# Jaureguy760/HaploHyped-VarAwareML

Hardware: AMD Instinct MI355X
Metric: variants/sec encode+compress, 3M-variant x 2.5k-sample VCF (higher is better)
Workload: dtype u8

## Files before the change

### haplohyped_varawareml_amd/csrc/api.hip

```cpp
#include "common.h"
#include <chrono>
#include <vector>
#include <stdarg.h>
#include <stdio.h>
#include <string.h>
#include <stdlib.h>

static thread_local char g_err[512] = "";

void hhgt_set_error(const char *fmt, ...)
{
    va_list ap;
    va_start(ap, fmt);
    vsnprintf(g_err, sizeof(g_err), fmt, ap);
    va_end(ap);
}

extern "C" const char *hhgt_last_error(void) { return g_err; }
extern "C" const char *hhgt_version(void) { return "hhgt 0.1 (gfx950)"; }

extern "C" int hhgt_device_count(void)
{
    int n = 0;
    if (hipGetDeviceCount(&n) != hipSuccess) return 0;
    return n;
}

int DevBuf::ensure(size_t bytes)
{
    if (bytes <= cap) return HHGT_OK;
    if (p) {
        hipFree(p);
        p = nullptr;
        cap = 0;
    }
    size_t want = bytes + bytes / 8 + 256;
    static const bool dbg = getenv("HHGT_ALLOC_DEBUG") != nullptr;
    const auto t0 = std::chrono::steady_clock::now();
    hipError_t e = hipMalloc(&p, want);
    if (dbg)
        fprintf(stderr, "[alloc] %.3f ms  hipMalloc %zu took %.3f ms\n", std::chrono::duration<double>(t0.time_since_epoch()).count() * 1e3,
                want, std::chrono::duration<double>(std::chrono::steady_clock::now() - t0).count() * 1e3);
    if (e != hipSuccess) {
        p = nullptr;
        hhgt_set_error("hipMalloc(%zu) failed: %s", want, hipGetErrorString(e));
        return HHGT_ERR_HIP;
    }
    cap = want;
    return HHGT_OK;
}

void DevBuf::release()
{
    if (p) hipFree(p);
    p = nullptr;
    cap = 0;
}

#define TRY(expr)                      \
    do {                               \
        int _rc = (expr);              \
        if (_rc != HHGT_OK) return _rc; \
    } while (0)

int EncodeWs::ensure_index(uint32_t n_regions)
{
    TRY(slots.ensure((size_t)n_regions * INDEX_CAP * 4));
    TRY(counts.ensure((size_t)n_regions * 4));
    TRY(prefix.ensure(((size_t)n_regions + 1) * 4));
    return ensure_scan(n_regions);
}

int EncodeWs::ensure_lines(uint32_t max_lines)
{
    const size_t nl4 = ((size_t)max_lines + 1) * 4;
    TRY(nl.ensure(nl4));
    TRY(ensure_scan(max_lines));
    for (DevBuf &b : line) TRY(b.ensure(nl4));
    return ensure_runs();
}

int EncodeWs::ensure_scan(uint64_t n) { return scan_tmp.ensure(2 * scan_tmp_elems(n) * 4); }

int EncodeWs::ensure_runs()
{
    TRY(run_first.ensure(MAX_CHROM_RUNS * 8));
    TRY(run_names.ensure(MAX_CHROM_RUNS * 32));
    return result.ensure(sizeof(hhgt_encode_result));
}

int hhgt_ctx::CodecWs::ensure(uint64_t n_chunks, uint32_t nblocks, uint32_t nwaves, size_t slot)
{
    const uint64_t n_streams = n_chunks * nblocks * nwaves;
    TRY(lz_scratch.ensure((size_t)n_streams * slot));
    TRY(lz_csize.ensure((size_t)n_streams * 4));
    TRY(fr_bsize.ensure((size_t)n_chunks * nblocks * 4));
    TRY(fr_csize.ensure(((size_t)n_chunks + 1) * 8));
    return fr_flags.ensure((size_t)n_chunks * 4);
}

template <typename Launch>
static int timed(hhgt_ctx *c, hipStream_t st, int stage, Launch launch)
{
    StageTimer t(c, st, stage);
    TRY(launch());
    t.stop();
    return HHGT_OK;
}

extern "C" int hhgt_ctx_create(int device, hhgt_ctx **out)
{
    if (!out) return HHGT_ERR_ARG;
    *out = nullptr;
    int n = hhgt_device_count();
    if (n <= 0 || device < 0 || device >= n) {
        hhgt_set_error("no usable HIP device (count=%d, requested=%d): libhhgt has no CPU path", n, device);
        return HHGT_ERR_NO_DEVICE;
    }
    HIP_TRY(hipSetDevice(device));
    hhgt_ctx *c = new hhgt_ctx();
    c->device = device;
    int rc = HHGT_OK;
    hipError_t e = hipGetDeviceProperties(&c->prop, device);
    if (e != hipSuccess) {
        hhgt_set_error("hipGetDeviceProperties failed: %s", hipGetErrorString(e));
        rc = HHGT_ERR_HIP;
    } else if (strncmp(c->prop.gcnArchName, "gfx950", 6) != 0) {
        hhgt_set_error("device %d is %s; libhhgt carries gfx950 code objects only", device, c->prop.gcnArchName);
        rc = HHGT_ERR_NO_DEVICE;
    }
    if (rc == HHGT_OK && (e = hipHostMalloc(reinterpret_cast<void **>(&c->h_counters), sizeof(DevCounters), hipHostMallocDefault)) != hipSuccess) {
        hhgt_set_error("hipHostMalloc failed: %s", hipGetErrorString(e));
        rc = HHGT_ERR_HIP;
    }
    if (rc == HHGT_OK && (e = hipHostMalloc(reinterpret_cast<void **>(&c->h_result_pinned), sizeof(hhgt_encode_result), hipHostMallocDefault)) != hipSuccess) {
        hhgt_set_error("hipHostMalloc failed: %s", hipGetErrorString(e));
        rc = HHGT_ERR_HIP;
    }
    if (rc == HHGT_OK) rc = c->counters.ensure(sizeof(DevCounters));
    if (rc != HHGT_OK) {
        hhgt_ctx_destroy(c);
        return rc;
    }
    *out = c;
    return HHGT_OK;
}

extern "C" void hhgt_ctx_destroy(hhgt_ctx *c)
{
    if (!c) return;
    hipSetDevice(c->device);
    hipDeviceSynchronize();
    c->enc.each([](DevBuf &b) { b.release(); });
    DevBuf *bufs[] = {&c->counters, &c->cursor, &c->dec_bad, &c->oh_ovl, &c->oh_lut, &c->crc_x2n, &c->ld_bits};
    for (DevBuf *b : bufs) b->release();
    for (auto &w : c->cw) {
        DevBuf *wb[] = {&w.lz_scratch, &w.lz_csize, &w.lz_flags, &w.fr_bsize, &w.fr_csize, &w.fr_flags};
        for (DevBuf *b : wb) b->release();
        if (w.lz_done) hipEventDestroy(w.lz_done);
        if (w.fr_done) hipEventDestroy(w.fr_done);
    }
    if (c->h_counters) hipHostFree(c->h_counters);
    if (c->h_result_pinned) hipHostFree(c->h_result_pinned);
    for (auto &p : c->pending) {
        hipEventDestroy(p.a);
        hipEventDestroy(p.b);
    }
    for (auto e : c->event_pool) hipEventDestroy(e);
    delete c;
}

static hipEvent_t get_event(hhgt_ctx *c)
{
    if (!c->event_pool.empty()) {
        hipEvent_t e = c->event_pool.back();
        c->event_pool.pop_back();
        return e;
    }
    hipEvent_t e;
    hipEventCreate(&e);
    return e;
}

StageTimer::StageTimer(hhgt_ctx *c, hipStream_t s, int stage_) : ctx(c), st(s), stage(stage_)
{
    if (ctx->profiling) {
        a = get_event(ctx);
        b = get_event(ctx);
        hipEventRecord(a, st);
    }
}

void StageTimer::stop()
{
    if (a) {
        hipEventRecord(b, st);
        ctx->pending.push_back({stage, a, b});
        a = b = nullptr;
    }
}

int hhgt_profile_collect(hhgt_ctx *c)
{
    for (auto &p : c->pending) {
        hipEventSynchronize(p.b);
        float ms = 0.f;
        if (hipEventElapsedTime(&ms, p.a, p.b) == hipSuccess) {
            c->stage_ms[p.stage] += ms;
            c->stage_launches[p.stage] += 1;
        }
        c->event_pool.push_back(p.a);
        c->event_pool.push_back(p.b);
    }
    c->pending.clear();
    return HHGT_OK;
}

extern "C" int hhgt_profile_enable(hhgt_ctx *c, int on)
{
    if (!c) return HHGT_ERR_ARG;
    c->profiling = on ? 1 : 0;
    return HHGT_OK;
}

extern "C" int hhgt_profile_reset(hhgt_ctx *c)
{
    if (!c) return HHGT_ERR_ARG;
    hhgt_profile_collect(c);
    for (int i = 0; i < HHGT_N_STAGES; ++i) {
        c->stage_ms[i] = 0;
        c->stage_launches[i] = 0;
    }
    return HHGT_OK;
}

extern "C" int hhgt_profile_read(hhgt_ctx *c, double *ms, uint64_t *launches)
{
    if (!c) return HHGT_ERR_ARG;
    hhgt_profile_collect(c);
    for (int i = 0; i < HHGT_N_STAGES; ++i) {
// ... 513 lines not shown
}

static int effective_blocksize(uint64_t chunk_nbytes, int typesize, int blocksize)
{
    if ((uint64_t)blocksize > chunk_nbytes) {
        blocksize = (int)chunk_nbytes;
        if (typesize > 1 && blocksize >= typesize) blocksize -= blocksize % typesize;
    }
    return blocksize > 0 ? blocksize : 1;
}

static int check_decode_block(int typesize, int blocksize)
{
    if (blocksize > 65536) {
        hhgt_set_error("decode: block of %d bytes x typesize %d does not fit LDS (blocks of at most 65536 bytes)",
                       blocksize, typesize);
        return HHGT_ERR_ARG;
    }
    return HHGT_OK;
}

static void codec_geometry(uint64_t chunk_nbytes, int typesize, int blocksize, uint32_t *nblocks, uint32_t *nwaves,
                           size_t *slot_bytes)
{
    const bool split = typesize >= 2 && typesize <= 16 && blocksize / typesize >= 128;
    *nblocks = (uint32_t)((chunk_nbytes + blocksize - 1) / blocksize);
    *nwaves = split ? (uint32_t)typesize : 1u;
    size_t max_stream = split ? (size_t)blocksize / typesize : (size_t)blocksize;
    if (split && chunk_nbytes % blocksize && chunk_nbytes % blocksize > max_stream) max_stream = chunk_nbytes % blocksize;
    *slot_bytes = lz4_slot_bytes((int)max_stream);
}

extern "C" uint64_t hhgt_compress_bound(uint64_t n_chunks, uint64_t chunk_nbytes, int typesize, int blocksize)
{
    if (check_codec_args(chunk_nbytes, typesize, blocksize, HHGT_BLOSC2) != HHGT_OK) return 0;
    return n_chunks * (chunk_nbytes + 32);
}

static int compress_impl(hhgt_ctx *c, const void *d_src, const void *d_planes, PlanesGeom pg, uint64_t n_chunks, uint64_t chunk_nbytes,
                         int typesize, int blocksize, int format, void *d_dst, uint64_t dst_cap,
                         uint64_t *d_chunk_off, uint64_t *total_bytes, void *stream)
{
    if (!c || (!d_src && !d_planes) || !d_dst || !d_chunk_off) return HHGT_ERR_ARG;
    hipStream_t st = reinterpret_cast<hipStream_t>(stream);
    HIP_TRY(hipSetDevice(c->device));
    TRY(check_codec_args(chunk_nbytes, typesize, blocksize, format));
    if (total_bytes) *total_bytes = 0;
    if (n_chunks == 0) return HHGT_OK;
    if (!total_bytes && dst_cap < n_chunks * (chunk_nbytes + 32)) {
        hhgt_set_error("compress: the asynchronous form (total_bytes == NULL) needs dst_cap >= hhgt_compress_bound() = %llu, got %llu",
                       (unsigned long long)(n_chunks * (chunk_nbytes + 32)), (unsigned long long)dst_cap);
        return HHGT_ERR_CAPACITY;
    }
    blocksize = effective_blocksize(chunk_nbytes, typesize, blocksize);
    uint32_t nblocks, nwaves;
    size_t slot;
    codec_geometry(chunk_nbytes, typesize, blocksize, &nblocks, &nwaves, &slot);
    hipStream_t fst = c->frame_stream ? c->frame_stream : st;
    hhgt_ctx::CodecWs &w = c->cw[c->frame_stream ? (c->cmp_seq++ & 1u) : 0u];
    TRY(w.ensure(n_chunks, nblocks, nwaves, slot));
    if (w.fr_pending) {
        HIP_TRY(hipStreamWaitEvent(st, w.fr_done, 0));
        w.fr_pending = false;
    }
    TRY(timed(c, st, HHGT_STAGE_LZ4, [&] {
        if (!w.lz_flags.p) {
            TRY(w.lz_flags.ensure(4));
            HIP_TRY(hipMemsetAsync(w.lz_flags.p, 0, 4, st));
        }
        if (++w.lz_tag == 0) w.lz_tag = 1;
        return launch_lz4_blocks(static_cast<const uint8_t *>(d_src), static_cast<const uint8_t *>(d_planes), pg, n_chunks, chunk_nbytes,
                                 typesize, blocksize, w.lz_scratch.as<uint8_t>(), slot, w.lz_csize.as<uint32_t>(), c->clevel,
                                 w.lz_flags.as<uint32_t>(), w.lz_tag, st);
    }));
    if (fst != st) {
        if (!w.lz_done) HIP_TRY(hipEventCreateWithFlags(&w.lz_done, hipEventDisableTiming));
        if (!w.fr_done) HIP_TRY(hipEventCreateWithFlags(&w.fr_done, hipEventDisableTiming));
        HIP_TRY(hipEventRecord(w.lz_done, st));
        HIP_TRY(hipStreamWaitEvent(fst, w.lz_done, 0));
    }
    TRY(timed(c, fst, HHGT_STAGE_FRAME, [&] {
        return launch_frame(w.lz_scratch.as<uint8_t>(), slot, w.lz_csize.as<uint32_t>(), static_cast<const uint8_t *>(d_src),
                            static_cast<const uint8_t *>(d_planes), pg, n_chunks, chunk_nbytes, typesize, blocksize, format,
                            w.fr_bsize.as<uint32_t>(), w.fr_csize.as<uint64_t>(), static_cast<uint8_t *>(d_dst), dst_cap, d_chunk_off,
                            w.fr_flags.as<uint32_t>(), fst);
    }));
    if (fst != st) {
        HIP_TRY(hipEventRecord(w.fr_done, fst));
        w.fr_pending = true;
        if (total_bytes) HIP_TRY(hipStreamWaitEvent(st, w.fr_done, 0));
    }
    if (total_bytes) {
        uint64_t tot = 0;
        HIP_TRY(hipMemcpyAsync(&tot, d_chunk_off + n_chunks, 8, hipMemcpyDeviceToHost, st));
        HIP_TRY(hipStreamSynchronize(st));
        *total_bytes = tot;
        if (tot > dst_cap) {
            hhgt_set_error("compress: need %llu bytes, dst_cap is %llu", (unsigned long long)tot,
                           (unsigned long long)dst_cap);
            return HHGT_ERR_CAPACITY;
        }
    }
    return HHGT_OK;
}

extern "C" int hhgt_compress_chunks(hhgt_ctx *c, const void *d_src, uint64_t n_chunks, uint64_t chunk_nbytes,
                                    int typesize, int blocksize, int format, void *d_dst, uint64_t dst_cap,
                                    uint64_t *d_chunk_off, uint64_t *total_bytes, void *stream)
{
    if (!d_src) return HHGT_ERR_ARG;
    return compress_impl(c, d_src, nullptr, PlanesGeom{0, 0, 0, 0}, n_chunks, chunk_nbytes, typesize, blocksize, format, d_dst, dst_cap,
                         d_chunk_off, total_bytes, stream);
}

extern "C" int hhgt_compress_planes(hhgt_ctx *c, const hhgt_layout *lay, const void *d_P, const void *d_G, uint32_t col0, uint32_t n_cols,
                                    int format, void *d_dst, uint64_t dst_cap, uint64_t *d_chunk_off, uint64_t *total_bytes,
                                    void *stream)
{
    if (!c || !d_P) return HHGT_ERR_ARG;
    LayoutDev L;
    PlanesGeom pg;
    TRY(planes_columns(lay, col0, n_cols, &L, &pg));
    const uint64_t chunk_nbytes = (uint64_t)L.Sc * L.Vc * 2ull, col_bytes = chunk_nbytes * L.n_sc;
    const uint8_t *g = d_G ? static_cast<const uint8_t *>(d_G) + (uint64_t)col0 * col_bytes : nullptr;
    return compress_impl(c, g, d_P, pg, (uint64_t)n_cols * L.n_sc, chunk_nbytes, 2, 8192, format, d_dst, dst_cap, d_chunk_off, total_bytes,
                         stream);
}

extern "C" int hhgt_reserve(hhgt_ctx *c, uint64_t text_bytes, uint32_t max_lines, uint64_t n_chunks, uint64_t chunk_nbytes, int typesize,
                            int blocksize)
{
    if (!c) return HHGT_ERR_ARG;
    HIP_TRY(hipSetDevice(c->device));
    if (text_bytes) {
        const uint32_t n_regions = index_regions(text_bytes);
        TRY(c->enc.ensure_scan(n_regions > max_lines ? n_regions : max_lines));
        TRY(c->enc.ensure_index(n_regions));
        TRY(c->enc.ensure_lines(max_lines));
    }
    if (n_chunks) {
        TRY(check_codec_args(chunk_nbytes, typesize, blocksize, HHGT_BLOSC2));
        blocksize = effective_blocksize(chunk_nbytes, typesize, blocksize);
        uint32_t nblocks, nwaves;
        size_t slot;
        codec_geometry(chunk_nbytes, typesize, blocksize, &nblocks, &nwaves, &slot);
        TRY(c->cw[0].ensure(n_chunks, nblocks, nwaves, slot));
    }
    return HHGT_OK;
}

extern "C" int hhgt_set_clevel(hhgt_ctx *c, int clevel)
{
    if (!c || clevel < 1 || clevel > 9) {
        hhgt_set_error("clevel must be 1..9");
        return HHGT_ERR_ARG;
    }
    c->clevel = clevel;
    return HHGT_OK;
}

extern "C" int hhgt_stream_create(hhgt_ctx *c, int kind, void **out)
{
    if (!c || !out || (kind != HHGT_STREAM_ENCODE && kind != HHGT_STREAM_COMPRESS && kind != HHGT_STREAM_FRAME)) {
        hhgt_set_error("hhgt_stream_create: bad arguments");
        return HHGT_ERR_ARG;
    }
    HIP_TRY(hipSetDevice(c->device));
    hipStream_t st = nullptr;
// ... 353 lines not shown
```

### haplohyped_varawareml_amd/csrc/common.h

```cpp
#pragma once
#include <hip/hip_runtime.h>
#include <stdint.h>
#include <stddef.h>
#include <string>
#include <vector>
#include "../../include/hhgt.h"

#define HHGT_WAVE 64
#ifdef HHGT_ENC_PRIO
#define HHGT_WAVE_PRIO() __builtin_amdgcn_s_setprio(HHGT_ENC_PRIO)
#else
#define HHGT_WAVE_PRIO()
#endif

#ifdef __HIPCC__
__device__ __forceinline__ uint32_t wave_scan_sum_dpp(uint32_t x, uint32_t lane)
{
    x += (uint32_t)__builtin_amdgcn_update_dpp(0, (int)x, 0x111, 0xf, 0xf, false);
    x += (uint32_t)__builtin_amdgcn_update_dpp(0, (int)x, 0x112, 0xf, 0xf, false);
    x += (uint32_t)__builtin_amdgcn_update_dpp(0, (int)x, 0x114, 0xf, 0xf, false);
    x += (uint32_t)__builtin_amdgcn_update_dpp(0, (int)x, 0x118, 0xf, 0xf, false);
    const uint32_t t0 = (uint32_t)__builtin_amdgcn_readlane((int)x, 15);
    const uint32_t t1 = (uint32_t)__builtin_amdgcn_readlane((int)x, 31) + t0;
    const uint32_t t2 = (uint32_t)__builtin_amdgcn_readlane((int)x, 47) + t1;
// ... 73 lines not shown
    uint32_t bpr;
    uint32_t tpc;
    uint32_t col0;
};
static inline __host__ __device__ uint64_t planes_piece(const PlanesGeom &g, uint64_t col, uint32_t tile, uint32_t kp, uint32_t row)
{
    return ((((col * g.tpc + tile) * 4ull + kp) * g.S_pad) + row) * 32ull;
}
static inline __host__ __device__ PlanesGeom planes_geom(const LayoutDev &L, uint32_t col0)
{
    PlanesGeom g;
    g.S_pad = L.n_sc * L.Sc;
    g.bpr = (uint32_t)(L.Vc >> 12);
    g.tpc = (uint32_t)(L.Vc / PL_TILE);
    g.col0 = col0;
    return g;
}
static inline __host__ __device__ void planes_block(const PlanesGeom &g, uint64_t id, uint64_t *col, uint32_t *row, uint32_t *bi)
{
    const uint64_t per_col = (uint64_t)g.S_pad * g.bpr;
    const uint64_t c = id / per_col;
    const uint32_t rem = (uint32_t)(id - c * per_col);
    *col = g.col0 + c;
    *row = rem / g.bpr;
    *bi = rem - (rem / g.bpr) * g.bpr;
}

struct DevBuf {
    void *p = nullptr;
    size_t cap = 0;
    int ensure(size_t bytes);
    void release();
    template <typename T> T *as() const { return reinterpret_cast<T *>(p); }
};

struct LineCols {
    uint32_t *soff, *lend, *pos, *refalt, *flags, *keep, *kidx, *cnew, *crun;
};
struct KeptCols {
    uint32_t *soff, *lend, *meta, *redo_list, *redo_flag;
    uint64_t *run_first;
    uint8_t *run_names;
};

struct EncodeWs {
    DevBuf slots, counts, prefix, nl, scan_tmp;
    enum { L_SOFF, L_LEND, L_POS, L_REFALT, L_FLAGS, L_KEEP, L_KIDX, L_CNEW, L_CRUN, K_SOFF, K_LEND, K_META, REDO_LIST, REDO_FLAG, N_LINE };
    DevBuf line[N_LINE];
    DevBuf run_first, run_names;
    DevBuf result;
    int ensure_index(uint32_t n_regions);
    int ensure_lines(uint32_t max_lines);
    int ensure_scan(uint64_t n);
    int ensure_runs();
    template <typename F> void each(F f)
    {
        for (DevBuf *b : {&slots, &counts, &prefix, &nl, &scan_tmp, &run_first, &run_names, &result}) f(*b);
        for (DevBuf &b : line) f(b);
    }
    uint32_t *col(int i) const { return line[i].as<uint32_t>(); }
    LineCols line_cols() const
    {
        LineCols l;
        l.soff = col(L_SOFF), l.lend = col(L_LEND), l.pos = col(L_POS), l.refalt = col(L_REFALT), l.flags = col(L_FLAGS);
        l.keep = col(L_KEEP), l.kidx = col(L_KIDX), l.cnew = col(L_CNEW), l.crun = col(L_CRUN);
        return l;
    }
    KeptCols kept_cols() const
    {
        KeptCols k;
        k.soff = col(K_SOFF), k.lend = col(K_LEND), k.meta = col(K_META), k.redo_list = col(REDO_LIST), k.redo_flag = col(REDO_FLAG);
        k.run_first = run_first.as<uint64_t>(), k.run_names = run_names.as<uint8_t>();
        return k;
    }
};

struct hhgt_ctx {
    int device = 0;
    hipDeviceProp_t prop;
    EncodeWs enc;
    DevBuf counters;
    DevBuf cursor;
    struct CodecWs {
        DevBuf lz_scratch, lz_csize, lz_flags, fr_bsize, fr_csize, fr_flags;
        uint32_t lz_tag = 0;
        hipEvent_t lz_done = nullptr, fr_done = nullptr;
        bool fr_pending = false;
        int ensure(uint64_t n_chunks, uint32_t nblocks, uint32_t nwaves, size_t slot);
    } cw[2];
    uint64_t cmp_seq = 0;
    hipStream_t frame_stream = nullptr;
    DevBuf dec_bad, oh_ovl, oh_lut, crc_x2n;
    DevBuf ld_bits;
    bool crc_x2n_ready = false;
    DevCounters *h_counters = nullptr;
    hhgt_encode_result *h_result_pinned = nullptr;
    hhgt_encode_result h_result;
    std::vector<uint64_t> run_first_kept;
    std::vector<std::string> run_names_host;
    int clevel = 5;
    int keep_multi = 0;
    int index_mode = -1;
    bool counters_clean = false;
    int profiling = 0;
    double stage_ms[HHGT_N_STAGES] = {0};
    uint64_t stage_launches[HHGT_N_STAGES] = {0};
    struct Pending { int stage; hipEvent_t a, b; };
    std::vector<Pending> pending;
    std::vector<hipEvent_t> event_pool;
};

struct StageTimer {
    hhgt_ctx *ctx;
    hipStream_t st;
    int stage;
    hipEvent_t a = nullptr, b = nullptr;
    StageTimer(hhgt_ctx *c, hipStream_t s, int stage_);
    void stop();
};
int hhgt_profile_collect(hhgt_ctx *ctx);

int launch_scan_exclusive_u32(const uint32_t *d_in, uint32_t *d_out, uint64_t n, uint32_t *d_tmp,
                              size_t tmp_elems, hipStream_t st);
int launch_scan_exclusive_u32_pair(const uint32_t *in_a, uint32_t *out_a, const uint32_t *in_b, uint32_t *out_b, uint64_t n,
                                   uint32_t *d_tmp, size_t tmp_elems, hipStream_t st);
size_t scan_tmp_elems(uint64_t n);

int launch_index_newlines(const uint8_t *d_text, uint64_t n, uint32_t *d_slots, uint32_t *d_counts,
                          uint32_t n_regions, uint32_t min_line, uint32_t S, int mode, DevCounters *d_cnt, hipStream_t st);
int index_mode_default();
int launch_compact_newlines(const uint32_t *d_slots, const uint32_t *d_counts, const uint32_t *d_prefix,
                            uint32_t n_regions, uint32_t *d_nl, uint32_t max_lines, hipStream_t st);
int launch_parse_fixed(const uint8_t *d_text, uint64_t n, const uint32_t *d_nl, const uint32_t *d_nlines,
                       uint32_t max_lines, const RegionFilter &region, uint32_t S, const LineCols &l, int mode,
                       DevCounters *d_cnt, hipStream_t st);
int launch_compact_kept(const uint8_t *d_text, uint64_t n, const uint32_t *d_nl, const uint32_t *d_nlines, uint32_t max_lines,
                        const LineCols &l, const KeptCols &k, uint32_t max_runs, const uint64_t *d_cursor, uint64_t v_capacity,
                        uint32_t ring, uint32_t *d_start, uint32_t *d_stop, uint8_t *d_ref, uint8_t *d_alt, DevCounters *d_cnt,
                        bool strided, hipStream_t st);

int launch_encode_tiles(const uint8_t *d_text, uint64_t n, const uint32_t *k_soff, const uint32_t *k_meta,
                        uint32_t n_lines_bound, const uint64_t *d_cursor, LayoutDev lay, int8_t *d_G,
                        uint32_t *redo_list, uint32_t *redo_flag, DevCounters *d_cnt, hipStream_t st);
int launch_encode_general(const uint8_t *d_text, uint64_t n, const uint32_t *k_soff, const uint32_t *k_lend,
                          const uint32_t *k_meta, const uint32_t *redo_list, const uint64_t *d_cursor, LayoutDev lay,
                          int8_t *d_G, uint8_t *d_P, DevCounters *d_cnt, int n_cu, hipStream_t st);
int launch_encode_planes(const uint8_t *d_text, uint64_t n, const uint32_t *k_soff, const uint32_t *k_meta,
                         uint32_t n_lines_bound, const uint64_t *d_cursor, LayoutDev lay, uint8_t *d_P, int8_t *d_G,
                         uint32_t *redo_list, uint32_t *redo_flag, DevCounters *d_cnt, hipStream_t st);
int launch_pad_tail_planes(LayoutDev lay, uint64_t v_end, uint64_t vcol_begin, uint64_t vcol_end, uint8_t *d_P, hipStream_t st);
int launch_pad_tail_planes_cursor(LayoutDev lay, const uint64_t *d_cursor, uint8_t *d_P, hipStream_t st);
int launch_planes_expand(LayoutDev lay, const uint8_t *d_P, const uint8_t *d_G, uint32_t col0, uint32_t n_cols, uint8_t *d_out, hipStream_t st);
int launch_pad_tail(LayoutDev lay, uint64_t v_end, uint64_t vcol_begin, uint64_t vcol_end, int8_t *d_G,
                    hipStream_t st);
int launch_pad_tail_cursor(LayoutDev lay, const uint64_t *d_cursor, int8_t *d_G, hipStream_t st);

size_t lz4_slot_bytes(int neblock);
int launch_lz4_blocks(const uint8_t *d_src, const uint8_t *d_planes, PlanesGeom pg, uint64_t n_chunks, uint64_t chunk_nbytes, int typesize,
                      int blocksize, uint8_t *d_scratch, size_t slot_bytes, uint32_t *d_csize, int clevel, uint32_t *d_flags, uint32_t tag,
                      hipStream_t st);
int launch_lz4_bitplanes(const uint8_t *d_src, bool planes, PlanesGeom pg, uint64_t n_blocks, uint8_t *d_scratch, size_t slot_bytes, uint32_t *d_csize,
                         int depth, uint32_t *d_flags, uint32_t tag, hipStream_t st);
int launch_frame(const uint8_t *d_scratch, size_t slot_bytes, const uint32_t *d_csize, const uint8_t *d_src, const uint8_t *d_planes,
                 PlanesGeom pg, uint64_t n_chunks, uint64_t chunk_nbytes, int typesize, int blocksize, int format,
                 uint32_t *d_bstart, uint64_t *d_chunk_csize, uint8_t *d_dst, uint64_t dst_cap,
                 uint64_t *d_chunk_off, uint32_t *d_chunk_flags, hipStream_t st);
int launch_decode(const uint8_t *d_src, const uint64_t *d_chunk_off, uint64_t n_chunks, uint64_t chunk_nbytes,
                  int typesize, int blocksize, uint8_t *d_dst, unsigned long long *d_bad, hipStream_t st);
int launch_decode_sel(const hhgt_block_sel *d_sel, uint32_t n_sel, uint64_t chunk_nbytes, int typesize, int blocksize,
                      uint8_t *d_dst, unsigned long long *d_bad, hipStream_t st);
int launch_count_alleles(const hhgt_count_sel *d_sel, uint32_t n_sel, uint32_t sc, uint32_t vc, int blocksize,
                         uint32_t *d_counts, uint64_t n_out, unsigned long long *d_bad, hipStream_t st);
int launch_count_samples(const hhgt_sample_sel *d_sel, uint32_t n_sel, uint32_t sc, uint32_t vc, int blocksize,
                         const uint32_t *d_vmask, uint64_t vmask_words, uint32_t *d_counts, uint64_t n_out,
                         unsigned long long *d_bad, hipStream_t st);
int launch_genotype_planes(const hhgt_plane_sel *d_sel, uint32_t n_sel, uint32_t sc, uint32_t vc, int blocksize,
                           const uint32_t *d_vmask, uint64_t vmask_words, uint32_t *d_planes, uint64_t n_rows,
                           uint64_t row_words, unsigned long long *d_bad, hipStream_t st);
int launch_pair_counts(const uint32_t *d_planes, uint32_t n_rows, uint64_t row_words, uint64_t w_lo, uint64_t w_hi,
                       uint32_t *d_table, hipStream_t st);
int launch_grm(const uint32_t *d_planes, uint32_t n_rows, uint64_t row_words, uint64_t w_lo, uint64_t w_hi, const float *d_z,
               double *d_table, hipStream_t st);
int launch_variant_planes(const uint32_t *d_planes, uint32_t n_rows, uint64_t row_words, uint64_t w_lo, uint64_t w_hi,
                          uint32_t *d_vplanes, hipStream_t st);
int launch_ld_counts(const uint32_t *d_vplanes, uint64_t n_var, uint64_t sw, uint32_t window, uint32_t *d_table,
                     hipStream_t st);
uint32_t ld_walk_words(uint32_t window);
int launch_ld_exceeds(const uint32_t *d_table, uint64_t n_var, uint32_t window, double r2, uint64_t *d_bits, hipStream_t st);
int launch_ld_walk(const uint64_t *d_bits, uint64_t n_var, uint32_t window, uint8_t *d_keep, hipStream_t st);
int launch_assoc_sums(const uint32_t *d_vplanes, uint64_t n_var, uint64_t sw, const double *d_w, uint32_t n_cols,
                      double *d_sums, hipStream_t st);
int launch_inflate(const uint8_t *d_src, uint64_t src_bytes, const uint64_t *d_comp_off, const uint32_t *d_comp_len,
                   const uint64_t *d_out_off, const uint32_t *d_isize, uint64_t n_members, uint8_t *d_dst,
                   uint64_t dst_bytes, uint32_t *d_status, const uint32_t *d_crc32, const uint32_t *d_x2n, hipStream_t st);
void crc32_x2n_table(uint32_t *t );

static inline __host__ __device__ uint64_t layout_offset(const LayoutDev &L, uint32_t s, uint64_t v)
{
    uint64_t vcol = v / L.Vc, vin = v - vcol * L.Vc;
    if (L.ring) vcol %= L.ring;
    uint32_t scol = (L.sc_log2 >= 31) ? 0u : (s >> L.sc_log2);
    uint32_t sin = s - scol * L.Sc;
    return (((vcol * L.n_sc + scol) * L.Sc + sin) * L.Vc + vin) * 2ull;
}
```

### haplohyped_varawareml_amd/csrc/frame.hip

```cpp
#include "common.h"

#define BLOSC_DOSHUFFLE 0x1u
#define BLOSC_MEMCPYED 0x2u
#define BLOSC_DOBITSHUFFLE 0x4u
#define BLOSC_DONT_SPLIT 0x10u

struct FrameParams {
    uint32_t nblocks, typesize, blocksize, split, nwaves, format, hl;
    uint64_t chunk_nbytes, slot_bytes;
};

__device__ __forceinline__ uint32_t frame_wave_incl_scan(uint32_t v)
{
    const int lane = threadIdx.x & 63;
#pragma unroll
    for (int d = 1; d < 64; d <<= 1) {
        uint32_t t = __shfl_up(v, d, 64);
        if (lane >= d) v += t;
    }
    return v;
}

__global__ __launch_bounds__(256) void k_frame_sizes(FrameParams P, const uint32_t *__restrict__ csize,
                                                     uint32_t *__restrict__ bstart,
                                                     unsigned long long *__restrict__ chunk_csize,
                                                     uint32_t *__restrict__ chunk_flags)
{
    __shared__ uint32_t sm[8];
    const uint64_t chunk = blockIdx.x;
    uint32_t carry = P.hl + 4u * P.nblocks;
    for (uint32_t b0 = 0; b0 < P.nblocks; b0 += 256u) {
        const uint32_t b = b0 + threadIdx.x;
        uint32_t sz = 0;
        if (b < P.nblocks) {
            const uint64_t boff = (uint64_t)b * P.blocksize;
            const bool leftover = P.chunk_nbytes - boff < P.blocksize;
            const uint32_t ns = (P.split && !leftover) ? P.typesize : 1u;
            const uint32_t *cs = csize + (chunk * P.nblocks + b) * P.nwaves;
            for (uint32_t j = 0; j < ns; ++j) sz += 4u + cs[j];
        }
        uint32_t inc = frame_wave_incl_scan(sz);
        const int lane = threadIdx.x & 63, w = threadIdx.x >> 6;
        if (lane == 63) sm[w] = inc;
        __syncthreads();
        uint32_t base = 0, tot = 0;
#pragma unroll
        for (int i = 0; i < 4; ++i) {
            uint32_t x = sm[i];
            if (i < w) base += x;
            tot += x;
        }
        __syncthreads();
        if (b < P.nblocks) bstart[chunk * P.nblocks + b] = carry + base + inc - sz;
        carry += tot;
    }
    if (threadIdx.x == 0) {
        uint32_t flags = 0;
        unsigned long long cb = carry;
        if (cb > P.chunk_nbytes + P.hl) {
            flags = 1u;
            cb = P.chunk_nbytes + P.hl;
        }
        chunk_csize[chunk] = cb;
        chunk_flags[chunk] = flags;
    }
}

__global__ __launch_bounds__(256) void k_scan_u64(const unsigned long long *__restrict__ in, uint64_t n,
                                                  unsigned long long *__restrict__ out)
{
    __shared__ unsigned long long sm[4];
    unsigned long long carry = 0;
    const int lane = threadIdx.x & 63, w = threadIdx.x >> 6;
    for (uint64_t i0 = 0; i0 < n; i0 += 256u) {
        const uint64_t i = i0 + threadIdx.x;
        unsigned long long v = i < n ? in[i] : 0ull, inc = v;
#pragma unroll
        for (int d = 1; d < 64; d <<= 1) {
            unsigned long long t = __shfl_up(inc, d, 64);
            if (lane >= d) inc += t;
        }
        if (lane == 63) sm[w] = inc;
        __syncthreads();
        unsigned long long base = 0, tot = 0;
#pragma unroll
        for (int k = 0; k < 4; ++k) {
            unsigned long long x = sm[k];
            if (k < w) base += x;
            tot += x;
        }
        __syncthreads();
        if (i < n) out[i] = carry + base + inc - v;
        carry += tot;
    }
    if (threadIdx.x == 0) out[n] = carry;
}

typedef uint32_t u32x4_fr __attribute__((ext_vector_type(4)));
typedef uint32_t u32x4_fr_unaligned __attribute__((ext_vector_type(4), aligned(1)));
struct WaveCopy {
    u32x4_fr a;
};

__device__ __forceinline__ void wave_copy_load(WaveCopy &c, const uint8_t *__restrict__ dst, const uint8_t *__restrict__ src,
                                               uint32_t n)
{
    const uint32_t o = (threadIdx.x & 63u) * 16u;
    c.a = u32x4_fr{0u, 0u, 0u, 0u};
    if (o < n) c.a = *reinterpret_cast<const u32x4_fr *>(src + o);
}

__device__ __forceinline__ void wave_put16(uint8_t *__restrict__ d, const u32x4_fr &v, uint32_t left)
{
    if (left >= 16u) {
        *reinterpret_cast<u32x4_fr_unaligned *>(d) = v;
        return;
    }
    const uint32_t w[4] = {v.x, v.y, v.z, v.w};
#pragma unroll
    for (uint32_t k = 0; k < 15u; ++k)
        if (k < left) d[k] = (uint8_t)(w[k >> 2] >> (8u * (k & 3u)));
}

__device__ __forceinline__ void wave_copy_store(const WaveCopy &c, uint8_t *__restrict__ dst, const uint8_t *__restrict__ src,
                                                uint32_t n)
{
    const uint32_t o = (threadIdx.x & 63u) * 16u;
    if (o < n) wave_put16(dst + o, c.a, n - o);
    for (uint32_t base = 1024u; base < n; base += 4096u) {
        u32x4_fr v[4];
#pragma unroll
        for (int k = 0; k < 4; ++k) {
            const uint32_t q = base + (uint32_t)k * 1024u + o;
            v[k] = u32x4_fr{0u, 0u, 0u, 0u};
            if (q < n) v[k] = *reinterpret_cast<const u32x4_fr *>(src + q);
        }
#pragma unroll
        for (int k = 0; k < 4; ++k) {
            const uint32_t q = base + (uint32_t)k * 1024u + o;
            if (q < n) wave_put16(dst + q, v[k], n - q);
        }
    }
}

__device__ __forceinline__ void wg_copy(uint8_t *__restrict__ dst, const uint8_t *__restrict__ src, uint32_t n)
{
    WaveCopy c;
    wave_copy_load(c, dst, src, n);
    wave_copy_store(c, dst, src, n);
}

__device__ __forceinline__ void frame_block(const FrameParams &P, const uint8_t *__restrict__ scratch, const uint32_t *__restrict__ csize,
                                            const uint8_t *__restrict__ src, uint8_t *__restrict__ dst, uint64_t chunk, uint32_t b,
                                            uint64_t gb, unsigned long long coff, unsigned long long cend, uint32_t memcpyed, uint32_t bs,
                                            const uint8_t *__restrict__ planes, const PlanesGeom &pg)
{
    const uint32_t lane = threadIdx.x & 63u;
    uint8_t *cdst = dst + coff;
    const uint32_t cbytes = (uint32_t)(cend - coff);
    if (b == 0 && lane < P.hl) {
        const uint32_t split_flag = P.split ? 0u : BLOSC_DONT_SPLIT;
        uint32_t flags = (1u << 5) | (P.typesize > 1u ? BLOSC_DOSHUFFLE : 0u) | split_flag | (memcpyed ? BLOSC_MEMCPYED : 0u);
        uint32_t i = lane;
        uint8_t v = 0;
        if (P.format == HHGT_BLOSC2) {
            if (i == 0) v = 5;
            else if (i == 1) v = 1;
            else if (i == 2) v = (uint8_t)(flags | BLOSC_DOSHUFFLE | BLOSC_DOBITSHUFFLE);
            else if (i == 3) v = (uint8_t)P.typesize;
            else if (i == 16 + 5) v = (flags & BLOSC_DOSHUFFLE) ? 1 : 0;
        } else {
            if (i == 0) v = 2;
            else if (i == 1) v = 1;
            else if (i == 2) v = (uint8_t)flags;
            else if (i == 3) v = (uint8_t)P.typesize;
        }
        if (i >= 4 && i < 8) v = (uint8_t)((uint32_t)P.chunk_nbytes >> ((i - 4) * 8));
        if (i >= 8 && i < 12) v = (uint8_t)(P.blocksize >> ((i - 8) * 8));
        if (i >= 12 && i < 16) v = (uint8_t)(cbytes >> ((i - 12) * 8));
        cdst[i] = v;
    }
    const uint64_t boff = (uint64_t)b * P.blocksize;
    const uint32_t bsize = (uint32_t)(P.chunk_nbytes - boff < P.blocksize ? P.chunk_nbytes - boff : P.blocksize);
    if (memcpyed) {
        const uint8_t *s = src + chunk * P.chunk_nbytes + boff;
        uint8_t *d = cdst + P.hl + boff;
        if (planes) {
            uint64_t pcol;
            uint32_t prow, pbi;
            planes_block(pg, gb, &pcol, &prow, &pbi);
            const uint64_t kst = (uint64_t)pg.S_pad * 32ull;
            for (uint32_t i = lane; i < 4096u; i += 64u) {
                const uint8_t *pl = planes + planes_piece(pg, pcol, pbi * 16u + (i >> 8), 0u, prow) + ((i & 255u) >> 3);
#pragma unroll
                for (uint32_t h = 0; h < 2u; ++h) {
                    uint32_t v = (pl[h * kst] >> (i & 7u)) & 1u;
                    if ((pl[(2ull + h) * kst] >> (i & 7u)) & 1u) v = v ? 0xF7u : (src ? (uint32_t)s[2u * i + h] : 0u);
                    d[2u * i + h] = (uint8_t)v;
                }
            }
        } else if ((reinterpret_cast<uintptr_t>(s) & 15u) == 0 && (bsize & 15u) == 0) wg_copy(d, s, bsize);
        else for (uint32_t i = lane; i < bsize; i += 64u) d[i] = s[i];
        return;
    }
    if (lane < 4) cdst[P.hl + 4u * b + lane] = (uint8_t)(bs >> (lane * 8));
    const bool leftover = bsize != P.blocksize;
    const uint32_t ns = (P.split && !leftover) ? P.typesize : 1u;
    uint32_t q = bs;
    const uint64_t sidx0 = ((uint64_t)chunk * P.nblocks + b) * P.nwaves;
    const uint32_t cs_l = lane < ns ? csize[sidx0 + lane] : 0u;
    if (ns == 2u) {
        const uint32_t cs0 = (uint32_t)__builtin_amdgcn_readlane((int)cs_l, 0), cs1 = (uint32_t)__builtin_amdgcn_readlane((int)cs_l, 1);
        uint8_t *d0 = cdst + q + 4u, *d1 = d0 + cs0 + 4u;
        const uint8_t *s0 = scratch + sidx0 * P.slot_bytes, *s1 = s0 + P.slot_bytes;
        WaveCopy c0, c1;
        wave_copy_load(c0, d0, s0, cs0);
        wave_copy_load(c1, d1, s1, cs1);
        if (lane < 4) cdst[q + lane] = (uint8_t)(cs0 >> (lane * 8));
        else if (lane < 8) d0[cs0 + lane - 4u] = (uint8_t)(cs1 >> ((lane - 4u) * 8));
        wave_copy_store(c0, d0, s0, cs0);
        wave_copy_store(c1, d1, s1, cs1);
        return;
    }
    for (uint32_t j = 0; j < ns; ++j) {
        const uint64_t sidx = sidx0 + j;
        const uint32_t cs = (uint32_t)__builtin_amdgcn_readlane((int)cs_l, (int)j);
        if (lane < 4) cdst[q + lane] = (uint8_t)(cs >> (lane * 8));
        wg_copy(cdst + q + 4u, scratch + sidx * P.slot_bytes, cs);
        q += 4u + cs;
    }
}

__global__ __launch_bounds__(256) void k_frame_write(FrameParams P, const uint8_t *__restrict__ scratch,
                                                     const uint32_t *__restrict__ csize,
                                                     const uint8_t *__restrict__ src,
                                                     const uint32_t *__restrict__ bstart,
                                                     const unsigned long long *__restrict__ chunk_off,
                                                     const uint32_t *__restrict__ chunk_flags,
                                                     uint8_t *__restrict__ dst, uint64_t dst_cap,
                                                     uint64_t n_total_blocks, const uint8_t *__restrict__ planes, PlanesGeom pg)
{
    const uint64_t gb = (uint64_t)blockIdx.x * (blockDim.x >> 6) + (threadIdx.x >> 6);
    if (gb >= n_total_blocks) return;
    const uint64_t chunk = gb / P.nblocks;
    const uint32_t b = (uint32_t)(gb - chunk * P.nblocks);
    const unsigned long long coff = chunk_off[chunk], cend = chunk_off[chunk + 1];
    if (cend > dst_cap) return;
    const uint32_t memcpyed = chunk_flags[chunk];
    frame_block(P, scratch, csize, src, dst, chunk, b, gb, coff, cend, memcpyed, memcpyed ? 0u : bstart[chunk * P.nblocks + b], planes, pg);
}

int launch_frame(const uint8_t *d_scratch, size_t slot_bytes, const uint32_t *d_csize, const uint8_t *d_src, const uint8_t *d_planes,
                 PlanesGeom pg, uint64_t n_chunks, uint64_t chunk_nbytes, int typesize, int blocksize, int format,
                 uint32_t *d_bstart, uint64_t *d_chunk_csize, uint8_t *d_dst, uint64_t dst_cap,
                 uint64_t *d_chunk_off, uint32_t *d_chunk_flags, hipStream_t st)
{
    if (n_chunks == 0) return HHGT_OK;
    FrameParams P;
    P.nblocks = (uint32_t)((chunk_nbytes + blocksize - 1) / blocksize);
    P.typesize = (uint32_t)typesize;
    P.blocksize = (uint32_t)blocksize;
    P.split = (typesize >= 2 && typesize <= 16 && blocksize / typesize >= 128) ? 1u : 0u;
    P.nwaves = P.split ? (uint32_t)typesize : 1u;
    P.format = (uint32_t)format;
    P.hl = format == HHGT_BLOSC2 ? 32u : 16u;
    P.chunk_nbytes = chunk_nbytes;
    P.slot_bytes = slot_bytes;
    hipLaunchKernelGGL(k_frame_sizes, dim3((uint32_t)n_chunks), dim3(256), 0, st, P, d_csize, d_bstart,
                       reinterpret_cast<unsigned long long *>(d_chunk_csize), d_chunk_flags);
    hipLaunchKernelGGL(k_scan_u64, dim3(1), dim3(256), 0, st,
                       reinterpret_cast<const unsigned long long *>(d_chunk_csize), n_chunks,
                       reinterpret_cast<unsigned long long *>(d_chunk_off));
    const uint64_t n_total_blocks = n_chunks * P.nblocks;
    hipLaunchKernelGGL(k_frame_write, dim3((uint32_t)((n_total_blocks + 3) / 4)), dim3(256), 0, st, P, d_scratch,
                       d_csize, d_src, d_bstart, reinterpret_cast<const unsigned long long *>(d_chunk_off),
                       d_chunk_flags, d_dst, dst_cap, n_total_blocks, d_planes, pg);
    HIP_TRY(hipGetLastError());
    return HHGT_OK;
}
```

Baseline: 152.4 million.

## Fuse frame size and chunk-offset scan kernels via last-block ticket

Merges the per-chunk size kernel and the single-block u64 scan kernel into one plan kernel. The last chunk block to finish, found with an atomicInc ticket, performs the offset scan. Per-block start, the first two stream sizes and the memcpy flag are packed into one 16-byte record so the write kernel does a single vector load instead of several scattered ones. The write kernel also raises wave priority. This removes one kernel launch and some dependent loads, at the cost of relying on atomic ticket and fence correctness and on the self-resetting counter.

Result: no change. 152.5 million (median of 3 runs) (+0.1%).

```diff
diff --git a/haplohyped_varawareml_amd/csrc/api.hip b/haplohyped_varawareml_amd/csrc/api.hip
--- a/haplohyped_varawareml_amd/csrc/api.hip
+++ b/haplohyped_varawareml_amd/csrc/api.hip
@@ -94,9 +94,12 @@
     const uint64_t n_streams = n_chunks * nblocks * nwaves;
     TRY(lz_scratch.ensure((size_t)n_streams * slot));
     TRY(lz_csize.ensure((size_t)n_streams * 4));
-    TRY(fr_bsize.ensure((size_t)n_chunks * nblocks * 4));
-    TRY(fr_csize.ensure(((size_t)n_chunks + 1) * 8));
-    return fr_flags.ensure((size_t)n_chunks * 4);
+    TRY(fr_rec.ensure((size_t)n_chunks * nblocks * 16));
+    const void *had = fr_tot.p;
+    const size_t had_cap = fr_tot.cap;
+    TRY(fr_tot.ensure(((size_t)n_chunks + 1) * 8));
+    if (fr_tot.p != had || fr_tot.cap != had_cap) HIP_TRY(hipMemset(fr_tot.p, 0, 8));
+    return HHGT_OK;
 }
 
 template <typename Launch>
@@ -155,7 +158,7 @@
     DevBuf *bufs[] = {&c->counters, &c->cursor, &c->dec_bad, &c->oh_ovl, &c->oh_lut, &c->crc_x2n, &c->ld_bits};
     for (DevBuf *b : bufs) b->release();
     for (auto &w : c->cw) {
-        DevBuf *wb[] = {&w.lz_scratch, &w.lz_csize, &w.lz_flags, &w.fr_bsize, &w.fr_csize, &w.fr_flags};
+        DevBuf *wb[] = {&w.lz_scratch, &w.lz_csize, &w.lz_flags, &w.fr_rec, &w.fr_tot};
         for (DevBuf *b : wb) b->release();
         if (w.lz_done) hipEventDestroy(w.lz_done);
         if (w.fr_done) hipEventDestroy(w.fr_done);
@@ -835,8 +838,7 @@
     TRY(timed(c, fst, HHGT_STAGE_FRAME, [&] {
         return launch_frame(w.lz_scratch.as<uint8_t>(), slot, w.lz_csize.as<uint32_t>(), static_cast<const uint8_t *>(d_src),
                             static_cast<const uint8_t *>(d_planes), pg, n_chunks, chunk_nbytes, typesize, blocksize, format,
-                            w.fr_bsize.as<uint32_t>(), w.fr_csize.as<uint64_t>(), static_cast<uint8_t *>(d_dst), dst_cap, d_chunk_off,
-                            w.fr_flags.as<uint32_t>(), fst);
+                            w.fr_rec.p, w.fr_tot.as<uint64_t>(), static_cast<uint8_t *>(d_dst), dst_cap, d_chunk_off, fst);
     }));
     if (fst != st) {
         HIP_TRY(hipEventRecord(w.fr_done, fst));
diff --git a/haplohyped_varawareml_amd/csrc/common.h b/haplohyped_varawareml_amd/csrc/common.h
--- a/haplohyped_varawareml_amd/csrc/common.h
+++ b/haplohyped_varawareml_amd/csrc/common.h
@@ -179,7 +179,9 @@
     DevBuf counters;
     DevBuf cursor;
     struct CodecWs {
-        DevBuf lz_scratch, lz_csize, lz_flags, fr_bsize, fr_csize, fr_flags;
+        DevBuf lz_scratch, lz_csize, lz_flags;
+        DevBuf fr_rec;
+        DevBuf fr_tot;
         uint32_t lz_tag = 0;
         hipEvent_t lz_done = nullptr, fr_done = nullptr;
         bool fr_pending = false;
@@ -260,8 +262,7 @@
                          int depth, uint32_t *d_flags, uint32_t tag, hipStream_t st);
 int launch_frame(const uint8_t *d_scratch, size_t slot_bytes, const uint32_t *d_csize, const uint8_t *d_src, const uint8_t *d_planes,
                  PlanesGeom pg, uint64_t n_chunks, uint64_t chunk_nbytes, int typesize, int blocksize, int format,
-                 uint32_t *d_bstart, uint64_t *d_chunk_csize, uint8_t *d_dst, uint64_t dst_cap,
-                 uint64_t *d_chunk_off, uint32_t *d_chunk_flags, hipStream_t st);
+                 void *d_rec, uint64_t *d_tot, uint8_t *d_dst, uint64_t dst_cap, uint64_t *d_chunk_off, hipStream_t st);
 int launch_decode(const uint8_t *d_src, const uint64_t *d_chunk_off, uint64_t n_chunks, uint64_t chunk_nbytes,
                   int typesize, int blocksize, uint8_t *d_dst, unsigned long long *d_bad, hipStream_t st);
 int launch_decode_sel(const hhgt_block_sel *d_sel, uint32_t n_sel, uint64_t chunk_nbytes, int typesize, int blocksize,
diff --git a/haplohyped_varawareml_amd/csrc/frame.hip b/haplohyped_varawareml_amd/csrc/frame.hip
--- a/haplohyped_varawareml_amd/csrc/frame.hip
+++ b/haplohyped_varawareml_amd/csrc/frame.hip
@@ -21,79 +21,91 @@
     return v;
 }
 
-__global__ __launch_bounds__(256) void k_frame_sizes(FrameParams P, const uint32_t *__restrict__ csize,
-                                                     uint32_t *__restrict__ bstart,
-                                                     unsigned long long *__restrict__ chunk_csize,
-                                                     uint32_t *__restrict__ chunk_flags)
+struct __attribute__((aligned(16))) BlockRec {
+    uint32_t bstart;
+    uint32_t cs0, cs1;
+    uint32_t memcpyed;
+};
+
+__global__ __launch_bounds__(256) void k_frame_plan(FrameParams P, const uint32_t *__restrict__ csize, BlockRec *__restrict__ rec,
+                                                    unsigned long long *tot, uint32_t n_chunks, unsigned long long *chunk_off)
 {
     __shared__ uint32_t sm[8];
+    __shared__ unsigned long long sm64[4];
+    __shared__ uint32_t s_last;
     const uint64_t chunk = blockIdx.x;
+    const int lane = threadIdx.x & 63, w = threadIdx.x >> 6;
     uint32_t carry = P.hl + 4u * P.nblocks;
     for (uint32_t b0 = 0; b0 < P.nblocks; b0 += 256u) {
         const uint32_t b = b0 + threadIdx.x;
-        uint32_t sz = 0;
+        uint32_t sz = 0, c0 = 0, c1 = 0;
         if (b < P.nblocks) {
             const uint64_t boff = (uint64_t)b * P.blocksize;
             const bool leftover = P.chunk_nbytes - boff < P.blocksize;
             const uint32_t ns = (P.split && !leftover) ? P.typesize : 1u;
             const uint32_t *cs = csize + (chunk * P.nblocks + b) * P.nwaves;
-            for (uint32_t j = 0; j < ns; ++j) sz += 4u + cs[j];
+            for (uint32_t j = 0; j < ns; ++j) {
+                const uint32_t c = cs[j];
+                if (j == 0) c0 = c;
+                if (j == 1) c1 = c;
+                sz += 4u + c;
+            }
         }
         uint32_t inc = frame_wave_incl_scan(sz);
-        const int lane = threadIdx.x & 63, w = threadIdx.x >> 6;
         if (lane == 63) sm[w] = inc;
         __syncthreads();
-        uint32_t base = 0, tot = 0;
+        uint32_t base = 0, tot_pass = 0;
 #pragma unroll
         for (int i = 0; i < 4; ++i) {
             uint32_t x = sm[i];
             if (i < w) base += x;
-            tot += x;
-        }
-        __syncthreads();
-        if (b < P.nblocks) bstart[chunk * P.nblocks + b] = carry + base + inc - sz;
-        carry += tot;
+            tot_pass += x;
+        }
+        __syncthreads();
+        if (b < P.nblocks) rec[chunk * P.nblocks + b] = BlockRec{carry + base + inc - sz, c0, c1, 0u};
+        carry += tot_pass;
+    }
+    unsigned long long cb = carry;
+    if (cb > P.chunk_nbytes + P.hl) {
+        cb = P.chunk_nbytes + P.hl;
+        for (uint32_t b = threadIdx.x; b < P.nblocks; b += 256u) rec[chunk * P.nblocks + b].memcpyed = 1u;
     }
     if (threadIdx.x == 0) {
-        uint32_t flags = 0;
-        unsigned long long cb = carry;
-        if (cb > P.chunk_nbytes + P.hl) {
-            flags = 1u;
-            cb = P.chunk_nbytes + P.hl;
-        }
-        chunk_csize[chunk] = cb;
-        chunk_flags[chunk] = flags;
-    }
-}
-
-__global__ __launch_bounds__(256) void k_scan_u64(const unsigned long long *__restrict__ in, uint64_t n,
-                                                  unsigned long long *__restrict__ out)
-{
-    __shared__ unsigned long long sm[4];
-    unsigned long long carry = 0;
-    const int lane = threadIdx.x & 63, w = threadIdx.x >> 6;
-    for (uint64_t i0 = 0; i0 < n; i0 += 256u) {
-        const uint64_t i = i0 + threadIdx.x;
-        unsigned long long v = i < n ? in[i] : 0ull, inc = v;
+        __hip_atomic_store(tot + 1 + chunk, cb, __ATOMIC_RELAXED, __HIP_MEMORY_SCOPE_AGENT);
+        asm volatile("s_waitcnt vmcnt(0)" ::: "memory");
+        const uint32_t ticket = atomicInc(reinterpret_cast<uint32_t *>(tot), n_chunks - 1u);
+        const bool last = ticket == n_chunks - 1u;
+        if (last) {
+            __builtin_amdgcn_fence(__ATOMIC_ACQUIRE, "agent");
+            asm volatile("s_waitcnt vmcnt(0)" ::: "memory");
+        }
+        s_last = last;
+    }
+    __syncthreads();
+    if (!s_last) return;
+    unsigned long long run = 0;
+    for (uint32_t i0 = 0; i0 < n_chunks; i0 += 256u) {
+        const uint32_t i = i0 + threadIdx.x;
+        unsigned long long v = i < n_chunks ? __hip_atomic_load(tot + 1 + i, __ATOMIC_RELAXED, __HIP_MEMORY_SCOPE_AGENT) : 0ull, inc = v;
 #pragma unroll
         for (int d = 1; d < 64; d <<= 1) {
             unsigned long long t = __shfl_up(inc, d, 64);
             if (lane >= d) inc += t;
         }
-        if (lane == 63) sm[w] = inc;
-        __syncthreads();
-        unsigned long long base = 0, tot = 0;
+        if (lane == 63) sm64[w] = inc;
+        __syncthreads();
+        unsigned long long base = 0, tot_pass = 0;
 #pragma unroll
         for (int k = 0; k < 4; ++k) {
-            unsigned long long x = sm[k];
+            unsigned long long x = sm64[k];
             if (k < w) base += x;
-            tot += x;
-        }
-        __syncthreads();
-        if (i < n) out[i] = carry + base + inc - v;
-        carry += tot;
-    }
-    if (threadIdx.x == 0) out[n] = carry;
+            tot_pass += x;
+        }
+        __syncthreads();
+        if (i < n_chunks) chunk_off[i] = run + base + inc - v;
+        run += tot_pass;
+    }
+    if (threadIdx.x == 0) chunk_off[n_chunks] = run;
 }
 
 typedef uint32_t u32x4_fr __attribute__((ext_vector_type(4)));
@@ -152,9 +164,10 @@
 
 __device__ __forceinline__ void frame_block(const FrameParams &P, const uint8_t *__restrict__ scratch, const uint32_t *__restrict__ csize,
                                             const uint8_t *__restrict__ src, uint8_t *__restrict__ dst, uint64_t chunk, uint32_t b,
-                                            uint64_t gb, unsigned long long coff, unsigned long long cend, uint32_t memcpyed, uint32_t bs,
+                                            uint64_t gb, unsigned long long coff, unsigned long long cend, const BlockRec &r,
                                             const uint8_t *__restrict__ planes, const PlanesGeom &pg)
 {
+    const uint32_t memcpyed = r.memcpyed, bs = r.bstart;
     const uint32_t lane = threadIdx.x & 63u;
     uint8_t *cdst = dst + coff;
     const uint32_t cbytes = (uint32_t)(cend - coff);
@@ -208,9 +221,8 @@
     const uint32_t ns = (P.split && !leftover) ? P.typesize : 1u;
     uint32_t q = bs;
     const uint64_t sidx0 = ((uint64_t)chunk * P.nblocks + b) * P.nwaves;
-    const uint32_t cs_l = lane < ns ? csize[sidx0 + lane] : 0u;
     if (ns == 2u) {
-        const uint32_t cs0 = (uint32_t)__builtin_amdgcn_readlane((int)cs_l, 0), cs1 = (uint32_t)__builtin_amdgcn_readlane((int)cs_l, 1);
+        const uint32_t cs0 = r.cs0, cs1 = r.cs1;
         uint8_t *d0 = cdst + q + 4u, *d1 = d0 + cs0 + 4u;
         const uint8_t *s0 = scratch + sidx0 * P.slot_bytes, *s1 = s0 + P.slot_bytes;
         WaveCopy c0, c1;
@@ -222,6 +234,7 @@
         wave_copy_store(c1, d1, s1, cs1);
         return;
     }
+    const uint32_t cs_l = lane < ns ? csize[sidx0 + lane] : 0u;
     for (uint32_t j = 0; j < ns; ++j) {
         const uint64_t sidx = sidx0 + j;
         const uint32_t cs = (uint32_t)__builtin_amdgcn_readlane((int)cs_l, (int)j);
@@ -234,26 +247,26 @@
 __global__ __launch_bounds__(256) void k_frame_write(FrameParams P, const uint8_t *__restrict__ scratch,
                                                      const uint32_t *__restrict__ csize,
                                                      const uint8_t *__restrict__ src,
-                                                     const uint32_t *__restrict__ bstart,
+                                                     const BlockRec *__restrict__ rec,
                                                      const unsigned long long *__restrict__ chunk_off,
-                                                     const uint32_t *__restrict__ chunk_flags,
                                                      uint8_t *__restrict__ dst, uint64_t dst_cap,
                                                      uint64_t n_total_blocks, const uint8_t *__restrict__ planes, PlanesGeom pg)
 {
+    __builtin_amdgcn_s_setprio(3);
     const uint64_t gb = (uint64_t)blockIdx.x * (blockDim.x >> 6) + (threadIdx.x >> 6);
     if (gb >= n_total_blocks) return;
     const uint64_t chunk = gb / P.nblocks;
     const uint32_t b = (uint32_t)(gb - chunk * P.nblocks);
-    const unsigned long long coff = chunk_off[chunk], cend = chunk_off[chunk + 1];
+    unsigned long long coff = chunk_off[chunk], cend = chunk_off[chunk + 1];
+    BlockRec r = rec[gb];
+    asm volatile("" : "+v"(coff), "+v"(cend), "+v"(r.bstart), "+v"(r.cs0), "+v"(r.cs1), "+v"(r.memcpyed));
     if (cend > dst_cap) return;
-    const uint32_t memcpyed = chunk_flags[chunk];
-    frame_block(P, scratch, csize, src, dst, chunk, b, gb, coff, cend, memcpyed, memcpyed ? 0u : bstart[chunk * P.nblocks + b], planes, pg);
+    frame_block(P, scratch, csize, src, dst, chunk, b, gb, coff, cend, r, planes, pg);
 }
 
 int launch_frame(const uint8_t *d_scratch, size_t slot_bytes, const uint32_t *d_csize, const uint8_t *d_src, const uint8_t *d_planes,
                  PlanesGeom pg, uint64_t n_chunks, uint64_t chunk_nbytes, int typesize, int blocksize, int format,
-                 uint32_t *d_bstart, uint64_t *d_chunk_csize, uint8_t *d_dst, uint64_t dst_cap,
-                 uint64_t *d_chunk_off, uint32_t *d_chunk_flags, hipStream_t st)
+                 void *d_rec, uint64_t *d_tot, uint8_t *d_dst, uint64_t dst_cap, uint64_t *d_chunk_off, hipStream_t st)
 {
     if (n_chunks == 0) return HHGT_OK;
     FrameParams P;
@@ -266,15 +279,14 @@
     P.hl = format == HHGT_BLOSC2 ? 32u : 16u;
     P.chunk_nbytes = chunk_nbytes;
     P.slot_bytes = slot_bytes;
-    hipLaunchKernelGGL(k_frame_sizes, dim3((uint32_t)n_chunks), dim3(256), 0, st, P, d_csize, d_bstart,
-                       reinterpret_cast<unsigned long long *>(d_chunk_csize), d_chunk_flags);
-    hipLaunchKernelGGL(k_scan_u64, dim3(1), dim3(256), 0, st,
-                       reinterpret_cast<const unsigned long long *>(d_chunk_csize), n_chunks,
+    BlockRec *rec = static_cast<BlockRec *>(d_rec);
+    hipLaunchKernelGGL(k_frame_plan, dim3((uint32_t)n_chunks), dim3(256), 0, st, P, d_csize, rec,
+                       reinterpret_cast<unsigned long long *>(d_tot), (uint32_t)n_chunks,
                        reinterpret_cast<unsigned long long *>(d_chunk_off));
     const uint64_t n_total_blocks = n_chunks * P.nblocks;
     hipLaunchKernelGGL(k_frame_write, dim3((uint32_t)((n_total_blocks + 3) / 4)), dim3(256), 0, st, P, d_scratch,
-                       d_csize, d_src, d_bstart, reinterpret_cast<const unsigned long long *>(d_chunk_off),
-                       d_chunk_flags, d_dst, dst_cap, n_total_blocks, d_planes, pg);
+                       d_csize, d_src, rec, reinterpret_cast<const unsigned long long *>(d_chunk_off),
+                       d_dst, dst_cap, n_total_blocks, d_planes, pg);
     HIP_TRY(hipGetLastError());
     return HHGT_OK;
 }
```
